# SciML/NeuralPDE.jl

Hardware: NVIDIA H100
Metric: collocation-points/sec (loss+grad) (higher is better)
Workload: dtype f32

## Files before the change

neuralpde.jl_b200/csrc/tc_kernel.cu:

```cuda
#include "tc_common.cuh"

namespace pinn {

using Fp = FpBlock<kTcW>;

struct CtaShared : CtaBase {
  int split, off_Q;
  uint8_t* stash;
  TcNetSmem nets[PINN_MAX_NETS];
};

struct LoopCtx {
  uint32_t fp;
  uint32_t bt;
  uint32_t tP;
  uint32_t tQ;
  float* gb;
  float* gw;
  uint32_t taddr;
  int act, split, p, lane, g0, g1, flag;
  __device__ __forceinline__ LoopCtx(uint32_t fp_, uint32_t bt_, uint32_t tP_, uint32_t tQ_, const Tid& t, int act_, int ng,
                                     int flag_, int split_ = 0, float* gb_ = nullptr, float* gw_ = nullptr)
      : fp(fp_), bt(bt_), tP(tP_), tQ(tQ_), gb(gb_), gw(gw_), taddr(t.lane_addr), act(act_), split(split_), p(t.p), lane(t.lane),
        g0(t.hh * (ng / kNH)), g1((t.hh + 1) * (ng / kNH)), flag(flag_) {}
};

template <int N1, int N2, bool PURE, int AK>
__device__ __forceinline__ void l0_fwd_loop(const LoopCtx lc, const PassInfo<N1, N2> pi, const float* xp, float* up) {
  constexpr int C = 1 + N1 + N2;
  float x[PINN_MAX_IN], u[C];
#pragma unroll
  for (int k = 0; k < PINN_MAX_IN; ++k) x[k] = xp[k];
#pragma unroll
  for (int c = 0; c < C; ++c) u[c] = up[c];
#pragma unroll 1
  for (int g = lc.g0; g < lc.g1; ++g) {
    float h[C][GW];
#pragma unroll
    for (int i = 0; i < GW; i += 2) {
      float za[C], zb2[C];
      first_layer_elem<kTcW>(lc.fp, pi, x, g * GW + i, za);
      first_layer_elem<kTcW>(lc.fp, pi, x, g * GW + i + 1, zb2);
      P2 zz[C], hv[C];
#pragma unroll
      for (int c = 0; c < C; ++c) zz[c] = mk2(za[c], zb2[c]);
      chain_fwd<N1, N2, PURE, AK, P2>(lc.act, pi.ch, zz, hv);
#pragma unroll
      for (int c = 0; c < C; ++c) { h[c][i] = hv[c].v.x; h[c][i + 1] = hv[c].v.y; }
      if (lc.flag) {
        const float w0 = lds_f32(lc.fp + (Fp::WL + g * GW + i) * 4), w1 = lds_f32(lc.fp + (Fp::WL + g * GW + i + 1) * 4);
#pragma unroll
        for (int c = 0; c < C; ++c) u[c] = fmaf(w1, hv[c].v.y, fmaf(w0, hv[c].v.x, u[c]));
      }
    }
#pragma unroll
    for (int c = 0; c < C; ++c) store_half(lc.tP + c * kTileBytes, lc.tQ + c * kTileBytes, lc.p, g * GW, h[c], lc.split != 0);
  }
#pragma unroll
  for (int c = 0; c < C; ++c) up[c] = u[c];
}

template <int C, int NK, bool SPLIT>
__device__ __forceinline__ void fwd_mma(float (&d)[C][16], uint32_t sP, uint32_t sQ, uint32_t whi, uint32_t wlo) {
  const int wg = threadIdx.x >> 7;
  const uint32_t aoff = (wg & 1) * 8192u, boff = (wg >> 1) * 32u * 128u;
  const uint64_t dwhi = tc::make_desc(whi + boff, 0, 1024), dwlo = tc::make_desc(wlo + boff, 0, 1024);
  tc::wgmma_fence();
#pragma unroll
  for (int c = 0; c < C; ++c) {
    const uint64_t dahi = tc::make_desc(sP + c * kTileBytes + aoff, 0, 1024);
    const uint64_t dalo = tc::make_desc(sQ + c * kTileBytes + aoff, 0, 1024);
#pragma unroll
    for (int pr = 0; pr < (SPLIT ? 3 : 1); ++pr) {
      const uint64_t a = (pr == 2) ? dalo : dahi, b = (pr == 1) ? dwlo : dwhi;
#pragma unroll
      for (int k = 0; k < NK; ++k)
        tc::wgmma_n32<0, 0>(d[c], a + 2 * k, b + 2 * k, (pr | k) ? 1u : 0u);
    }
  }
  tc::wgmma_commit();
  tc::wgmma_wait0();
}
template <int C>
__device__ __forceinline__ void fwd_mma_any(float (&d)[C][16], uint32_t sP, uint32_t sQ, uint32_t whi, uint32_t wlo, int nk,
                                            bool split) {
  switch (nk * 2 + (split ? 1 : 0)) {
    case 2: fwd_mma<C, 1, false>(d, sP, sQ, whi, wlo); break;
    case 3: fwd_mma<C, 1, true>(d, sP, sQ, whi, wlo); break;
    case 4: fwd_mma<C, 2, false>(d, sP, sQ, whi, wlo); break;
    case 5: fwd_mma<C, 2, true>(d, sP, sQ, whi, wlo); break;
    case 6: fwd_mma<C, 3, false>(d, sP, sQ, whi, wlo); break;
    case 7: fwd_mma<C, 3, true>(d, sP, sQ, whi, wlo); break;
    case 8: fwd_mma<C, 4, false>(d, sP, sQ, whi, wlo); break;
    default: fwd_mma<C, 4, true>(d, sP, sQ, whi, wlo); break;
  }
}

template <int N1, int N2, bool PURE, int AK, int C>
__device__ __forceinline__ void tl_fwd_frag(const float (&d)[C][16], const LoopCtx lc, const Chan<N1, N2> ch, float* scratch) {
  const int wg = threadIdx.x >> 7, w = (threadIdx.x >> 5) & 3;
  const int row0 = 64 * (wg & 1) + 16 * w + (lc.lane >> 2);
  const int col0 = 32 * (wg >> 1) + 2 * (lc.lane & 3);
  float u[2][C];
#pragma unroll
  for (int r = 0; r < 2; ++r)
#pragma unroll
    for (int c = 0; c < C; ++c) u[r][c] = 0.f;
#pragma unroll
  for (int i = 0; i < 16; i += 2) {
    const int rh = (i >> 1) & 1;
    const int row = row0 + 8 * rh, col = col0 + 8 * (i >> 2);
    P2 zz[C], hv[C];
    zz[0] = mk2(d[0][i] + lds_f32(lc.bt + col * 4), d[0][i + 1] + lds_f32(lc.bt + (col + 1) * 4));
#pragma unroll
    for (int c = 1; c < C; ++c) zz[c] = mk2(d[c][i], d[c][i + 1]);
    chain_fwd<N1, N2, PURE, AK, P2>(lc.act, ch, zz, hv);
    const uint32_t off = tc::swz_off(row, col);
#pragma unroll
    for (int c = 0; c < C; ++c) {
      const uint32_t hx = tc::pack_bf16(hv[c].v.x, hv[c].v.y);
      asm volatile("st.shared.b32 [%0], %1;" ::"r"(lc.tP + c * kTileBytes + off), "r"(hx) : "memory");
      if (lc.split)
        asm volatile("st.shared.b32 [%0], %1;" ::"r"(lc.tQ + c * kTileBytes + off), "r"(bf16x2_lo(hv[c].v.x, hv[c].v.y, hx))
                     : "memory");
    }
    if (lc.flag) {
      const float w0 = lds_f32(lc.fp + (Fp::WL + col) * 4), w1 = lds_f32(lc.fp + (Fp::WL + col + 1) * 4);
#pragma unroll
      for (int c = 0; c < C; ++c) u[rh][c] = fmaf(w1, hv[c].v.y, fmaf(w0, hv[c].v.x, u[rh][c]));
    }
  }
  if (lc.flag) {
#pragma unroll
    for (int r = 0; r < 2; ++r)
#pragma unroll
      for (int c = 0; c < C; ++c) {
        float s = u[r][c];
        s += __shfl_xor_sync(0xffffffffu, s, 1);
        s += __shfl_xor_sync(0xffffffffu, s, 2);
        if ((lc.lane & 3) == 0) atomicAdd(&scratch[c * kTcPts + row0 + 8 * r], s);
      }
  }
}

template <int C, int NKO>
__device__ __forceinline__ void dgrad_mma(float (&d)[C][16], uint32_t sP, uint32_t whi) {
  const uint32_t poff = (threadIdx.x >> 7) * 32u * 128u;
  const uint64_t dw = tc::make_desc(whi, 0, 1024);
  tc::wgmma_fence();
#pragma unroll
  for (int c = 0; c < C; ++c) {
    const uint64_t dz = tc::make_desc(sP + c * kTileBytes + poff, 0, 1024);
#pragma unroll
    for (int k = 0; k < NKO; ++k)
      tc::wgmma_n32<1, 0>(d[c], dw + 128 * k, dz + 2 * k, k ? 1u : 0u);
  }
  tc::wgmma_commit();
  tc::wgmma_wait0();
}
template <int C>
__device__ __forceinline__ void dgrad_mma_any(float (&d)[C][16], uint32_t sP, uint32_t whi, int nko) {
  switch (nko) {
    case 1: dgrad_mma<C, 1>(d, sP, whi); break;
    case 2: dgrad_mma<C, 2>(d, sP, whi); break;
    case 3: dgrad_mma<C, 3>(d, sP, whi); break;
    default: dgrad_mma<C, 4>(d, sP, whi); break;
  }
}
template <int C>
__device__ __forceinline__ void wgrad_mma(float (&dw)[32], float (&db)[8], uint32_t sP, uint32_t sQ, uint32_t s_ones) {
  const uint32_t poff = (threadIdx.x >> 7) * 32u * 128u;
  const uint64_t d1 = tc::make_desc(s_ones, 0, 0);
  tc::wgmma_fence();
#pragma unroll
  for (int c = 0; c < C; ++c) {
    const uint64_t dh = tc::make_desc(sQ + c * kTileBytes + poff, 0, 1024), dz = tc::make_desc(sP + c * kTileBytes + poff, 0, 1024);
#pragma unroll
    for (int k = 0; k < 2; ++k) tc::wgmma_n64<1, 1>(dw, dh + 128 * k, dz + 128 * k, (c | k) ? 1u : 0u);
  }
  const uint64_t dz0 = tc::make_desc(sP + poff, 0, 1024);
#pragma unroll
  for (int k = 0; k < 2; ++k) tc::wgmma_n16<1, 1>(db, dz0 + 128 * k, d1, k ? 1u : 0u);
  tc::wgmma_commit();
  tc::wgmma_wait0();
}

template <int NF>
__device__ __forceinline__ void frag_store_rows(float* base, int ld, const float (&d)[NF]) {
  const int w = (threadIdx.x >> 5) & 3, lane = threadIdx.x & 31;
  const bool odd = (lane & 1) != 0;
  float* row = base + (16 * w + (lane >> 2) + (odd ? 8 : 0)) * ld + 4 * ((lane >> 1) & 1);
#pragma unroll
  for (int j = 0; j < NF / 4; ++j) {
    const float r0 = __shfl_xor_sync(0xffffffffu, odd ? d[4 * j] : d[4 * j + 2], 1);
    const float r1 = __shfl_xor_sync(0xffffffffu, odd ? d[4 * j + 1] : d[4 * j + 3], 1);
    *reinterpret_cast<float4*>(row + 8 * j) =
        odd ? make_float4(r0, r1, d[4 * j + 2], d[4 * j + 3]) : make_float4(d[4 * j], d[4 * j + 1], r0, r1);
  }
}

template <int N1, int N2, bool PURE, int AK, int C>
__device__ __forceinline__ void tl_bwd_frag(const float (&d)[C][16], const LoopCtx lc, const Chan<N1, N2> ch, const float* ubs) {
  const int wg = threadIdx.x >> 7, w = (threadIdx.x >> 5) & 3;
  const int row0 = 64 * (wg & 1) + 16 * w + (lc.lane >> 2);
  const int col0 = 32 * (wg >> 1) + 2 * (lc.lane & 3);
  const float* hbar = tc::s_acc + TM_X * kAccRows;
#pragma unroll
  for (int i = 0; i < 16; i += 2) {
    const int row = row0 + 8 * ((i >> 1) & 1), col = col0 + 8 * (i >> 2);
    P2 zz[C], hv[C], zv[C];
    zz[0] = mk2(d[0][i] + lds_f32(lc.bt + col * 4), d[0][i + 1] + lds_f32(lc.bt + (col + 1) * 4));
#pragma unroll
    for (int c = 1; c < C; ++c) zz[c] = mk2(d[c][i], d[c][i + 1]);
    if (lc.flag) {
      const float w0 = lds_f32(lc.fp + (Fp::WL + col) * 4), w1 = lds_f32(lc.fp + (Fp::WL + col + 1) * 4);
#pragma unroll
      for (int c = 0; c < C; ++c) {
        const float u = ubs[c * kTcPts + row];
        hv[c] = mk2(w0 * u, w1 * u);
      }
    } else {
#pragma unroll
      for (int c = 0; c < C; ++c) hv[c] = mk2(hbar[(c * 64 + col) * kAccRows + row], hbar[(c * 64 + col + 1) * kAccRows + row]);
    }
    chain_bwd<N1, N2, PURE, AK, P2>(lc.act, ch, zz, hv, zv);
    const uint32_t off = tc::swz_off(row, col);
#pragma unroll
    for (int c = 0; c < C; ++c)
      asm volatile("st.shared.b32 [%0], %1;" ::"r"(lc.tP + c * kTileBytes + off), "r"(tc::pack_bf16(zv[c].v.x, zv[c].v.y))
                   : "memory");
  }
}

template <int N1, int N2, bool PURE, int AK>
__device__ __forceinline__ void l0_bwd_store_loop(const LoopCtx lc, const PassInfo<N1, N2> pi, const float* xp) {
  constexpr int C = 1 + N1 + N2;
  float x[PINN_MAX_IN];
#pragma unroll
  for (int k = 0; k < PINN_MAX_IN; ++k) x[k] = xp[k];
#pragma unroll 1
  for (int g = lc.g0; g < lc.g1; ++g) {
    float hb[C][GWB];
#pragma unroll
    for (int c = 0; c < C; ++c) acc_ldg(lc.taddr + TM_X + c * 64 + g * GWB, hb[c]);
#pragma unroll
    for (int i = 0; i < GWB; i += 2) {
      float za[C], zb2[C];
      first_layer_elem<kTcW>(lc.fp, pi, x, g * GWB + i, za);
      first_layer_elem<kTcW>(lc.fp, pi, x, g * GWB + i + 1, zb2);
      P2 zz[C], hv[C], zv[C];
#pragma unroll
      for (int c = 0; c < C; ++c) { zz[c] = mk2(za[c], zb2[c]); hv[c] = mk2(hb[c][i], hb[c][i + 1]); }
      chain_bwd<N1, N2, PURE, AK, P2>(lc.act, pi.ch, zz, hv, zv);
#pragma unroll
      for (int c = 0; c <= N1; ++c) { hb[c][i] = zv[c].v.x; hb[c][i + 1] = zv[c].v.y; }
    }
#pragma unroll
    for (int c = 0; c <= N1; ++c) store_half(lc.tP + c * kTileBytes, lc.tP, lc.p, g * GWB, hb[c], false);
  }
}

template <int N1, int N2, bool PURE, int AK>
__device__ __forceinline__ void l0_bwd_loop(const LoopCtx lc, const PassInfo<N1, N2> pi, const float* xp, const float* ubp) {
  constexpr int C = 1 + N1 + N2;
  float x[PINN_MAX_IN], ub[C];
#pragma unroll
  for (int k = 0; k < PINN_MAX_IN; ++k) x[k] = xp[k];
#pragma unroll
  for (int c = 0; c < C; ++c) ub[c] = ubp[c];
  const int re = reduceg_elem(lc.lane);
  const bool rlead = reduceg_lead(lc.lane);
  const int n1w = pi.n1w;
#pragma unroll 1
  for (int g = lc.g0; g < lc.g1; ++g) {
    float hb[C][GW];
    if (!lc.flag) {
#pragma unroll
      for (int c = 0; c < C; ++c) acc_ldg(lc.taddr + TM_X + c * 64 + g * GW, hb[c]);
    } else {
#pragma unroll
      for (int i = 0; i < GW; ++i) {
        const float wl = lds_f32(lc.fp + (Fp::WL + g * GW + i) * 4);
#pragma unroll
        for (int c = 0; c < C; ++c) hb[c][i] = wl * ub[c];
      }
    }
    float zv0[GW], zvd[N1 > 0 ? N1 : 1][GW];
#pragma unroll
    for (int i = 0; i < GW; ++i) {
      float zz[C], hv[C], zv[C];
      first_layer_elem<kTcW>(lc.fp, pi, x, g * GW + i, zz);
#pragma unroll
      for (int c = 0; c < C; ++c) hv[c] = hb[c][i];
      chain_bwd<N1, N2, PURE, AK, float>(lc.act, pi.ch, zz, hv, zv);
      zv0[i] = zv[0];
#pragma unroll
      for (int jd = 0; jd < N1; ++jd) zvd[jd][i] = zv[1 + jd];
    }
    const float bs = warp_reduceg(zv0, lc.lane);
    if (rlead) atomicAdd(lc.gb + g * GW + re, bs);
#pragma unroll
    for (int k = 0; k < PINN_MAX_IN; ++k) {
      if (k < pi.d_in) {
        float gk[GW];
#pragma unroll
        for (int i = 0; i < GW; ++i) {
          float gg = zv0[i] * x[k];
#pragma unroll
          for (int jd = 0; jd < N1; ++jd) gg += (pi.dir1[jd] == k) ? zvd[jd][i] : 0.f;
          gk[i] = gg;
        }
        const float gs = warp_reduceg(gk, lc.lane);
        if (rlead) atomicAdd(lc.gw + g * GW + re + (long long)n1w * k, gs);
      }
    }
  }
}

template <int N1, int N2, bool PURE, int AK>
__device__ __noinline__ uint32_t net_forward(CtaShared* cs, const DevProblem* Pp, const DevTerm* tmp, int slot,
                                             int want_grad, uint32_t phase) {
  extern __shared__ __align__(1024) uint8_t smem[];
  constexpr int C = 1 + N1 + N2;
  const DevTerm& tm = *tmp;
  const int net_id = tm.used_net[slot];
  const DevNet& net = Pp->nets[net_id];
  const DevChan& dc = tm.chan[slot];
  const TcNetSmem ns = cs->nets[net_id];
  const float* fp = reinterpret_cast<const float*>(smem + ns.fp);
  uint8_t* tP = smem + cs->off_P;
  uint8_t* tQ = smem + cs->off_Q;
  const Misc ms = misc_of(smem + cs->off_misc, cs->mx_dim, cs->mx_taps);
  const uint32_t accm = 0;
  const bool split = cs->split != 0;
  PassInfo<N1, N2> pi;
  load_pass<N1, N2>(pi, net, dc);
  const int TL = pi.TL;
  const Tid t = tid_of();
  const int tid = t.tid, p = t.p;
  float x[PINN_MAX_IN];
#pragma unroll
  for (int k = 0; k < PINN_MAX_IN; ++k) x[k] = (k < pi.d_in) ? ms.Xs[dc.rows[k] * kTcPts + p] : 0.f;
  uint8_t* stash_slot = cs->stash + (size_t)slot * cs->tl_max * kTcMaxC * kTileBytes;

  dbg_mark(cs, 10);
  float u[C];
#pragma unroll
  for (int c = 0; c < C; ++c) u[c] = 0.f;
  if (tid < C * kTcPts / 4) reinterpret_cast<float4*>(ms.scratch)[tid] = make_float4(0.f, 0.f, 0.f, 0.f);
  {
    const LoopCtx lc(tc::smem_u32(fp), tc::smem_u32(fp), tc::smem_u32(tP), tc::smem_u32(tQ), t, net.acts[0], pi.n1w / GW, TL == 0, split);
    l0_fwd_loop<N1, N2, PURE, AK>(lc, pi, x, u);
  }
  for (int l = 1; l <= TL; ++l) {
    const int n_in = net.dims[l], n_out = net.dims[l + 1];
    const int act = net.acts[l];
    tc::fence_async_smem();
    __syncthreads();
    dbg_mark(cs, 11);
    if (want_grad && tid == 0) {
      for (int c = 0; c < C; ++c)
        tc::bulk_store(stash_slot + (size_t)(l - 1) * kTcMaxC * kTileBytes + (size_t)c * kTileBytes, tP + c * kTileBytes, kTileBytes);
      tc::bulk_commit();
    }
    float d[C][16];
    {
      const uint32_t sP = tc::smem_u32(tP), sQ = tc::smem_u32(tQ);
      const uint32_t whi = tc::smem_u32(smem + ns.w_hi[l - 1]), wlo = tc::smem_u32(smem + ns.w_lo[l - 1]);
      const int nk = n_in / 16;
      fwd_mma_any<C>(d, sP, sQ, whi, wlo, nk, split);
    }
    dbg_mark(cs, 13);
    if (want_grad && tid == 0) tc::bulk_wait_read0();
    __syncthreads();
    dbg_mark(cs, 14);
    const LoopCtx lc(tc::smem_u32(fp), tc::smem_u32(fp) + (Fp::BT + (l - 1) * 64) * 4, tc::smem_u32(tP), tc::smem_u32(tQ), t, act, 0, l == TL, split);
    tl_fwd_frag<N1, N2, PURE, AK, C>(d, lc, pi.ch, ms.scratch);
  }
  finish_forward<C>(cs, tm, slot, ms, fp + Fp::BL, t, u);
  return phase;
}

template <int N1, int N2, bool PURE, int AK>
__device__ __noinline__ uint32_t net_backward(CtaShared* cs, const DevProblem* Pp, const DevTerm* tmp, int slot,
                                              uint32_t phase) {
  extern __shared__ __align__(1024) uint8_t smem[];
  constexpr int C = 1 + N1 + N2;
  const DevTerm& tm = *tmp;
  const int net_id = tm.used_net[slot];
  const DevNet& net = Pp->nets[net_id];
  const DevChan& dc = tm.chan[slot];
  const TcNetSmem ns = cs->nets[net_id];
  const float* fp = reinterpret_cast<const float*>(smem + ns.fp);
  uint8_t* tP = smem + cs->off_P;
  uint8_t* tQ = smem + cs->off_Q;
  const Misc ms = misc_of(smem + cs->off_misc, cs->mx_dim, cs->mx_taps);
  const uint32_t accm = 0;
  float* partial = cs->partial;
  PassInfo<N1, N2> pi;
  load_pass<N1, N2>(pi, net, dc);
  const int L = pi.L, TL = pi.TL;
  const Tid t = tid_of();
  const int tid = t.tid, p = t.p;
  uint32_t ld_phase = (phase >> 1) & 1u;
  float x[PINN_MAX_IN];
#pragma unroll
  for (int k = 0; k < PINN_MAX_IN; ++k) x[k] = (k < pi.d_in) ? ms.Xs[dc.rows[k] * kTcPts + p] : 0.f;
  uint8_t* stash_slot = cs->stash + (size_t)slot * cs->tl_max * kTcMaxC * kTileBytes;

  dbg_mark(cs, 20);
  float ub[C];
  gather_ubar<C>(tm, slot, ms, p, ub);
  if (t.hh == 0) {
#pragma unroll
    for (int c = 0; c < C; ++c) ms.scratch[c * kTcPts + p] = ub[c];
  }
  last_layer_grad<C>(t, ub, pi.nL, partial + net.w_off[L - 1], partial + net.b_off[L - 1], tc::smem_u32(tQ), tc::smem_u32(tP),
                     kTileBytes, 0u, accm + TM_Y, kTcW);

  const uint32_t sP = tc::smem_u32(tP), sQ = tc::smem_u32(tQ);
  const int wg = tid >> 7;
  float* hand = tc::s_acc + TM_X * kAccRows;
  float* wpart = reinterpret_cast<float*>(tP);
  float* bpart = ms.scratch;
  static_assert(4 * 64 <= kTcMaxC * kTcPts, "the bias partials fit ms.scratch");
  for (int l = TL; l >= 1; --l) {
    const int n_in = net.dims[l], n_out = net.dims[l + 1];
    const int act = net.acts[l];
    float* gb = partial + net.b_off[l];
    float* gw = partial + net.w_off[l];
    const float* bt = fp + Fp::BT + (l - 1) * 64;
    const uint32_t whi = tc::smem_u32(smem + ns.w_hi[l - 1]);
    dbg_mark(cs, 21);
    if (tid == 0 && l == TL) {
      const uint8_t* src = stash_slot + (size_t)(l - 1) * kTcMaxC * kTileBytes;
      tc::mbar_arrive_expect_tx(ms.bar_ld, C * kTileBytes);
      for (int c = 0; c < C; ++c) tc::bulk_load(tQ + c * kTileBytes, src + (size_t)c * kTileBytes, kTileBytes, ms.bar_ld);
    }
    wait_bar(ms.bar_ld, ld_phase);
    dbg_mark(cs, 22);
    {
      float d[C][16];
      fwd_mma_any<C>(d, sQ, sQ, whi, whi, n_in / 16, false);
      __syncthreads();
      dbg_mark(cs, 24);
      const LoopCtx lc(tc::smem_u32(fp), tc::smem_u32(bt), sP, sQ, t, act, 0, l == TL);
      tl_bwd_frag<N1, N2, PURE, AK, C>(d, lc, pi.ch, ms.scratch);
    }
    tc::fence_async_smem();
    __syncthreads();
    dbg_mark(cs, 26);
    {
      float d[C][16];
      dgrad_mma_any<C>(d, sP, whi, n_out / 16);
#pragma unroll
      for (int c = 0; c < C; ++c) frag_store_rows(hand + c * 64 * kAccRows + 32 * wg, kAccRows, d[c]);
    }
    dbg_mark(cs, 27);
    {
      float dw[32], db[8];
      wgrad_mma<C>(dw, db, sP, sQ, tc::smem_u32(smem + cs->off_ones));
      __syncthreads();
      if (tid == 0 && l > 1) {
        const uint8_t* src = stash_slot + (size_t)(l - 2) * kTcMaxC * kTileBytes;
        tc::mbar_arrive_expect_tx(ms.bar_ld, C * kTileBytes);
        for (int c = 0; c < C; ++c) tc::bulk_load(tQ + c * kTileBytes, src + (size_t)c * kTileBytes, kTileBytes, ms.bar_ld);
      }
      frag_store_rows(wpart + wg * 64 * 64, 64, dw);
      if ((t.lane & 3) == 0) {
        const int o = 16 * (t.warp & 3) + (t.lane >> 2);
        bpart[wg * 64 + o] = db[0];
        bpart[wg * 64 + o + 8] = db[2];
      }
    }
    __syncthreads();
    dbg_mark(cs, 28);
#pragma unroll 1
    for (int e = tid; e < 64 * 64; e += kTcThreads) {
      const int k = e >> 6, o = e & 63;
      if (k < n_in && o < n_out) atomicAdd(gw + o + (long long)n_out * k, ((wpart[e] + wpart[4096 + e]) + wpart[8192 + e]) + wpart[12288 + e]);
    }
    if (tid < n_out) atomicAdd(gb + tid, ((bpart[tid] + bpart[64 + tid]) + bpart[128 + tid]) + bpart[192 + tid]);
  }

  {
    __syncthreads();
    dbg_mark(cs, 29);
    const int act0 = net.acts[0];
    float* gb0 = partial + net.b_off[0];
    float* gw0 = partial + net.w_off[0];
    if (TL == 0) {
      const LoopCtx lc(tc::smem_u32(fp), tc::smem_u32(fp), sP, sQ, t, act0, pi.n1w / GW, 1, 0, gb0, gw0);
      l0_bwd_loop<N1, N2, PURE, AK>(lc, pi, x, ub);
    } else {
      coord_tiles<N1>(t, sQ, x, pi.dir1, N2 > 0);
      const LoopCtx lc(tc::smem_u32(fp), tc::smem_u32(fp), sP, sQ, t, act0, pi.n1w / GWB, 0);
      l0_bwd_store_loop<N1, N2, PURE, AK>(lc, pi, x);
      layer0_grad<N1>(t, sP, kTileBytes, 0u, sQ, N2 > 0, accm + TM_Y, kTcW, pi.n1w, pi.d_in, gw0, gb0);
    }
  }
  __syncthreads();
  dbg_mark(cs, 30);
  return (ld_phase << 1) | (phase & 1u);
}


__global__ void __launch_bounds__(kTcThreads, 1) tc_loss_grad_kernel(const __grid_constant__ TcArgs args) {
  extern __shared__ __align__(1024) uint8_t smem[];
  __shared__ CtaShared cs;
  const int tid = threadIdx.x;
  const DevProblem* Pp = args.prob;
  const DevProblem& P = *Pp;
  const Misc ms = misc_of(smem + args.off_misc, args.mx_dim, args.mx_taps);
  float* partial = args.partial + (long long)blockIdx.x * args.partial_stride;
  const bool want_grad = (args.mode == 0);
  const float* theta = args.theta;
  const DbgSpan span = dbg_span_begin(args.dbg);

  for (long long i = (long long)tid * 32; i < args.n_theta; i += (long long)kTcThreads * 32) tc::prefetch_l2(theta + i);
  {
    const char* nets0 = reinterpret_cast<const char*>(&Pp->nets[0]);
    const char* terms0 = reinterpret_cast<const char*>(&Pp->terms[0]);
    const int nb_nets = args.n_nets * (int)sizeof(DevNet), nb_terms = args.n_terms * (int)sizeof(DevTerm);
    if (tid == 0) tc::prefetch_l2(Pp);
    for (int o = tid * 128; o < nb_nets; o += kTcThreads * 128) tc::prefetch_l2(nets0 + o);
    for (int o = tid * 128; o < nb_terms; o += kTcThreads * 128) tc::prefetch_l2(terms0 + o);
    const int tile = args.tile_begin + (int)blockIdx.x;
    if (tile < args.tile_end && tid < 32) {
      int ti = 0;
      while (ti + 1 < args.n_terms && tile >= args.dyn[ti + 1].tile0) ++ti;
      const long long p0 = (long long)(tile - args.dyn[ti].tile0) * kTcPts;
      const long long row_bytes = 4ll * args.term_dim[ti];
      const long long off = p0 * row_bytes + (long long)tid * 128;
      if (off < args.dyn[ti].n * row_bytes) tc::prefetch_l2(reinterpret_cast<const char*>(args.dyn[ti].pts) + off);
    }
  }
  if (tid == 0) {
    tc::mbar_init(ms.bar_ld, 1);
    tc::fence_barrier_init();
    cs.split = args.split; cs.off_Q = args.off_Q;
    cs.stash = args.stash + (long long)blockIdx.x * args.stash_per_cta;
    for (int k = 0; k < PINN_MAX_NETS; ++k) cs.nets[k] = args.nets[k];
    cta_base_init(cs, args, partial);
  }
  if (tid == 0) tc::s_acc = args.acc + (size_t)blockIdx.x * kAccCols * kAccRows;
  cta_setup(args, ms, partial, P.n_theta, want_grad);
  for (int kn = 0; kn < P.n_nets; ++kn) {
    const DevNet& net = P.nets[kn];
    const TcNetSmem& ns = args.nets[kn];
    if (ns.fp < 0) continue;
    stage_fp_block<kTcW>(reinterpret_cast<float*>(smem + ns.fp), net, theta);
    const int L = net.n_layers;
    {
      constexpr int kItMax = kTcMaxTL * 512 / kTcThreads;
      const int n_items = (L - 2) * 512;
      float w[kItMax][8];
#pragma unroll
      for (int it = 0; it < kItMax; ++it) {
        const int i = tid + it * kTcThreads;
        if (i < n_items) {
          const int l = 1 + i / 512, r = i & 511;
          const int o = r & 63, kc = r >> 6;
          const int n_in = net.dims[l], n_out = net.dims[l + 1];
          const long long woff = net.w_off[l];
#pragma unroll
          for (int e = 0; e < 8; ++e) {
            const int k = kc * 8 + e;
            w[it][e] = (o < n_out && k < n_in) ? __ldg(&theta[woff + o + (long long)n_out * k]) : 0.f;
          }
        }
      }
#pragma unroll
      for (int it = 0; it < kItMax; ++it) {
        const int i = tid + it * kTcThreads;
        if (i < n_items) {
          const int l = 1 + i / 512, r = i & 511;
          const int o = r & 63, kc = r >> 6;
          uint8_t* thi = smem + ns.w_hi[l - 1];
          uint8_t* tlo = smem + ns.w_lo[l - 1];
          const float* v = w[it];
          uint32_t h[4];
#pragma unroll
          for (int e = 0; e < 4; ++e) h[e] = tc::pack_bf16(v[2 * e], v[2 * e + 1]);
          *reinterpret_cast<uint4*>(thi + tc::swz_chunk(o, kc)) = make_uint4(h[0], h[1], h[2], h[3]);
          if (args.split)
            *reinterpret_cast<uint4*>(tlo + tc::swz_chunk(o, kc)) = make_uint4(
                bf16x2_lo(v[0], v[1], h[0]), bf16x2_lo(v[2], v[3], h[1]), bf16x2_lo(v[4], v[5], h[2]), bf16x2_lo(v[6], v[7], h[3]));
        }
      }
    }
  }
  tc::fence_async_smem();
  __syncthreads();
  dbg_mark(&cs, 2);
  uint32_t phase = 0;

  for (int tile = args.tile_begin + blockIdx.x; tile < args.tile_end; tile += gridDim.x) {
    if (tid >= 128 && tid < 128 + (int)((sizeof(DevNet) * PINN_MAX_NETS + 127) / 128))
      tc::prefetch_l1(reinterpret_cast<const char*>(&P.nets[0]) + (tid - 128) * 128);
    uint32_t ldp = (phase >> 1) & 1u;
    const TileRef tr = stage_tile(args, P, ms, tile, ldp);
    phase = (phase & 1u) | (ldp << 1);
    const DevTerm* tmp = &P.terms[tr.ti];
    const DevTerm& tm = *tmp;
    const int n_used = tm.n_used;
    dbg_mark(&cs, 3);

    for (int slot = 0; slot < n_used; ++slot) {
      const int k1 = tm.chan[slot].n1, k2 = tm.chan[slot].n2, pu = tm.chan[slot].pure;
      const int ak = args.net_ak[tm.used_net[slot]];
      PINN_TC_DISPATCH(kTcMaxC, k1, k2, pu, ak, (phase = net_forward<A1, A2, PU, AK>(&cs, Pp, tmp, slot, want_grad ? 1 : 0, phase)));
    }

    dbg_mark(&cs, 4);
    residual_step(args, P, tm, ms, tr, smem + args.off_Q, (size_t)args.off_Q_bytes, partial, want_grad);

    dbg_mark(&cs, 5);
    if (want_grad) {
      if (tid == 0) tc::bulk_wait0();
      __syncthreads();
      dbg_mark(&cs, 6);
      for (int slot = n_used - 1; slot >= 0; --slot) {
        const int k1 = tm.chan[slot].n1, k2 = tm.chan[slot].n2, pu = tm.chan[slot].pure;
        const int ak = args.net_ak[tm.used_net[slot]];
        if (n_used > 1) {
          PINN_TC_DISPATCH(kTcMaxC, k1, k2, pu, ak, (phase = net_forward<A1, A2, PU, AK>(&cs, Pp, tmp, slot, 0, phase)));
        }
        PINN_TC_DISPATCH(kTcMaxC, k1, k2, pu, ak, (phase = net_backward<A1, A2, PU, AK>(&cs, Pp, tmp, slot, phase)));
      }
    }
  }

  __syncthreads();
  dbg_mark(&cs, 7);
  cta_finish(args, cs, span, ms, P, want_grad);
}

size_t tc_misc_bytes(int mx_dim, int mx_taps) {
  return (size_t)mx_dim * kTcPts * 4 + 2 * (size_t)mx_taps * kTcPts * 4 + (size_t)kTcMaxC * kTcPts * 4 + kTcPts * 4 +
         PINN_MAX_TERMS * 8 + 16 + 16;
}

cudaError_t tc_launch(const TcArgs& a, int grid, size_t smem, cudaStream_t st) {
  return launch_fused_kernel<tc_loss_grad_kernel>(a, grid, kTcThreads, smem, st);
}

}
```

Measured before the change: 93.04 million.

## Split hidden-layer backward into two 64-point halves reusing tile buffers

Restructures the hidden-layer backward pass to process the 128 collocation points in two halves. Each half recomputes its forward pre-activations with narrower n16 wgmma, writes the backward z into the second half of the Q tile, and keeps hbar in a swizzled smem layout inside the freed P tile. The weight-gradient partials now use plain (vectorised float4) read-modify-write into the per-CTA partial buffer instead of atomics, and the layer-0 path for TL==0 is hoisted. The intent is to cut shared-memory footprint and the number of bulk-load bytes per step and to remove atomic traffic, at the cost of twice as many layer iterations and barriers.

```diff
diff --git a/neuralpde.jl_b200/csrc/tc_kernel.cu b/neuralpde.jl_b200/csrc/tc_kernel.cu
--- a/neuralpde.jl_b200/csrc/tc_kernel.cu
+++ b/neuralpde.jl_b200/csrc/tc_kernel.cu
@@ -143,46 +143,94 @@
   }
 }
 
+constexpr uint32_t kHalfBytes = kTileBytes / 2;
+
+template <int C, int NK>
+__device__ __forceinline__ void rec_mma(float (&d)[C][8], uint32_t sQ, uint32_t whi) {
+  const uint64_t dw = tc::make_desc(whi + (threadIdx.x >> 7) * 16u * 128u, 0, 1024);
+  tc::wgmma_fence();
+#pragma unroll
+  for (int c = 0; c < C; ++c) {
+    const uint64_t da = tc::make_desc(sQ + c * kTileBytes, 0, 1024);
+#pragma unroll
+    for (int k = 0; k < NK; ++k) tc::wgmma_n16<0, 0>(d[c], da + 2 * k, dw + 2 * k, k ? 1u : 0u);
+  }
+  tc::wgmma_commit();
+  tc::wgmma_wait0();
+}
+template <int C>
+__device__ __forceinline__ void rec_mma_any(float (&d)[C][8], uint32_t sQ, uint32_t whi, int nk) {
+  switch (nk) {
+    case 1: rec_mma<C, 1>(d, sQ, whi); break;
+    case 2: rec_mma<C, 2>(d, sQ, whi); break;
+    case 3: rec_mma<C, 3>(d, sQ, whi); break;
+    default: rec_mma<C, 4>(d, sQ, whi); break;
+  }
+}
 template <int C, int NKO>
-__device__ __forceinline__ void dgrad_mma(float (&d)[C][16], uint32_t sP, uint32_t whi) {
-  const uint32_t poff = (threadIdx.x >> 7) * 32u * 128u;
+__device__ __forceinline__ void dgrad_mma(float (&d)[C][8], uint32_t sQ, uint32_t whi) {
+  const uint32_t poff = kHalfBytes + (threadIdx.x >> 7) * 16u * 128u;
   const uint64_t dw = tc::make_desc(whi, 0, 1024);
   tc::wgmma_fence();
 #pragma unroll
   for (int c = 0; c < C; ++c) {
-    const uint64_t dz = tc::make_desc(sP + c * kTileBytes + poff, 0, 1024);
+    const uint64_t dz = tc::make_desc(sQ + c * kTileBytes + poff, 0, 1024);
 #pragma unroll
     for (int k = 0; k < NKO; ++k)
-      tc::wgmma_n32<1, 0>(d[c], dw + 128 * k, dz + 2 * k, k ? 1u : 0u);
+      tc::wgmma_n16<1, 0>(d[c], dw + 128 * k, dz + 2 * k, k ? 1u : 0u);
   }
   tc::wgmma_commit();
   tc::wgmma_wait0();
 }
 template <int C>
-__device__ __forceinline__ void dgrad_mma_any(float (&d)[C][16], uint32_t sP, uint32_t whi, int nko) {
+__device__ __forceinline__ void dgrad_mma_any(float (&d)[C][8], uint32_t sQ, uint32_t whi, int nko) {
   switch (nko) {
-    case 1: dgrad_mma<C, 1>(d, sP, whi); break;
-    case 2: dgrad_mma<C, 2>(d, sP, whi); break;
-    case 3: dgrad_mma<C, 3>(d, sP, whi); break;
-    default: dgrad_mma<C, 4>(d, sP, whi); break;
+    case 1: dgrad_mma<C, 1>(d, sQ, whi); break;
+    case 2: dgrad_mma<C, 2>(d, sQ, whi); break;
+    case 3: dgrad_mma<C, 3>(d, sQ, whi); break;
+    default: dgrad_mma<C, 4>(d, sQ, whi); break;
   }
 }
 template <int C>
-__device__ __forceinline__ void wgrad_mma(float (&dw)[32], float (&db)[8], uint32_t sP, uint32_t sQ, uint32_t s_ones) {
-  const uint32_t poff = (threadIdx.x >> 7) * 32u * 128u;
+__device__ __forceinline__ void wgrad_mma(float (&dw)[32], float (&db)[8], uint32_t sQ, uint32_t s_ones) {
+  const uint32_t poff = (threadIdx.x >> 7) * 16u * 128u;
   const uint64_t d1 = tc::make_desc(s_ones, 0, 0);
   tc::wgmma_fence();
 #pragma unroll
   for (int c = 0; c < C; ++c) {
-    const uint64_t dh = tc::make_desc(sQ + c * kTileBytes + poff, 0, 1024), dz = tc::make_desc(sP + c * kTileBytes + poff, 0, 1024);
-#pragma unroll
-    for (int k = 0; k < 2; ++k) tc::wgmma_n64<1, 1>(dw, dh + 128 * k, dz + 128 * k, (c | k) ? 1u : 0u);
-  }
-  const uint64_t dz0 = tc::make_desc(sP + poff, 0, 1024);
-#pragma unroll
-  for (int k = 0; k < 2; ++k) tc::wgmma_n16<1, 1>(db, dz0 + 128 * k, d1, k ? 1u : 0u);
+    const uint64_t dh = tc::make_desc(sQ + c * kTileBytes + poff, 0, 1024);
+    const uint64_t dz = tc::make_desc(sQ + c * kTileBytes + kHalfBytes + poff, 0, 1024);
+    tc::wgmma_n64<1, 1>(dw, dh, dz, c ? 1u : 0u);
+  }
+  tc::wgmma_n16<1, 1>(db, tc::make_desc(sQ + kHalfBytes + poff, 0, 1024), d1, 0u);
   tc::wgmma_commit();
   tc::wgmma_wait0();
+}
+
+__device__ __forceinline__ int hb_idx(int c, int k, int p) { return (c * 64 + k) * 64 + (p ^ ((((k >> 1) ^ k) & 3) << 3)); }
+
+template <int C>
+__device__ __forceinline__ void hbar_store(float* hbar, const float (&d)[C][8]) {
+  const int wg = threadIdx.x >> 7, w = (threadIdx.x >> 5) & 3, lane = threadIdx.x & 31;
+#pragma unroll
+  for (int c = 0; c < C; ++c)
+#pragma unroll
+    for (int i = 0; i < 8; i += 2) {
+      const int k = 16 * w + (lane >> 2) + 8 * ((i >> 1) & 1), p = 16 * wg + 8 * (i >> 2) + 2 * (lane & 3);
+      *reinterpret_cast<float2*>(hbar + hb_idx(c, k, p)) = make_float2(d[c][i], d[c][i + 1]);
+    }
+}
+
+template <int C>
+__device__ __forceinline__ void hbar0_store(float* hand, const float (&d)[C][8], int h) {
+  const int wg = threadIdx.x >> 7, w = (threadIdx.x >> 5) & 3, lane = threadIdx.x & 31;
+#pragma unroll
+  for (int c = 0; c < C; ++c)
+#pragma unroll
+    for (int i = 0; i < 8; i += 2) {
+      const int k = 16 * w + (lane >> 2) + 8 * ((i >> 1) & 1), p = 64 * h + 16 * wg + 8 * (i >> 2) + 2 * (lane & 3);
+      *reinterpret_cast<float2*>(hand + (c * 64 + k) * kAccRows + p) = make_float2(d[c][i], d[c][i + 1]);
+    }
 }
 
 template <int NF>
@@ -200,13 +248,13 @@
 }
 
 template <int N1, int N2, bool PURE, int AK, int C>
-__device__ __forceinline__ void tl_bwd_frag(const float (&d)[C][16], const LoopCtx lc, const Chan<N1, N2> ch, const float* ubs) {
+__device__ __forceinline__ void tl_bwd_frag(const float (&d)[C][8], const LoopCtx lc, const Chan<N1, N2> ch, const float* ubs,
+                                            const float* hbar, int h) {
   const int wg = threadIdx.x >> 7, w = (threadIdx.x >> 5) & 3;
-  const int row0 = 64 * (wg & 1) + 16 * w + (lc.lane >> 2);
-  const int col0 = 32 * (wg >> 1) + 2 * (lc.lane & 3);
-  const float* hbar = tc::s_acc + TM_X * kAccRows;
-#pragma unroll
-  for (int i = 0; i < 16; i += 2) {
+  const int row0 = 16 * w + (lc.lane >> 2);
+  const int col0 = 16 * wg + 2 * (lc.lane & 3);
+#pragma unroll
+  for (int i = 0; i < 8; i += 2) {
     const int row = row0 + 8 * ((i >> 1) & 1), col = col0 + 8 * (i >> 2);
     P2 zz[C], hv[C], zv[C];
     zz[0] = mk2(d[0][i] + lds_f32(lc.bt + col * 4), d[0][i + 1] + lds_f32(lc.bt + (col + 1) * 4));
@@ -216,18 +264,18 @@
       const float w0 = lds_f32(lc.fp + (Fp::WL + col) * 4), w1 = lds_f32(lc.fp + (Fp::WL + col + 1) * 4);
 #pragma unroll
       for (int c = 0; c < C; ++c) {
-        const float u = ubs[c * kTcPts + row];
+        const float u = ubs[c * kTcPts + 64 * h + row];
         hv[c] = mk2(w0 * u, w1 * u);
       }
     } else {
 #pragma unroll
-      for (int c = 0; c < C; ++c) hv[c] = mk2(hbar[(c * 64 + col) * kAccRows + row], hbar[(c * 64 + col + 1) * kAccRows + row]);
+      for (int c = 0; c < C; ++c) hv[c] = mk2(hbar[hb_idx(c, col, row)], hbar[hb_idx(c, col + 1, row)]);
     }
     chain_bwd<N1, N2, PURE, AK, P2>(lc.act, ch, zz, hv, zv);
-    const uint32_t off = tc::swz_off(row, col);
+    const uint32_t off = kHalfBytes + tc::swz_off(row, col);
 #pragma unroll
     for (int c = 0; c < C; ++c)
-      asm volatile("st.shared.b32 [%0], %1;" ::"r"(lc.tP + c * kTileBytes + off), "r"(tc::pack_bf16(zv[c].v.x, zv[c].v.y))
+      asm volatile("st.shared.b32 [%0], %1;" ::"r"(lc.tQ + c * kTileBytes + off), "r"(tc::pack_bf16(zv[c].v.x, zv[c].v.y))
                    : "memory");
   }
 }
@@ -274,16 +322,11 @@
 #pragma unroll 1
   for (int g = lc.g0; g < lc.g1; ++g) {
     float hb[C][GW];
-    if (!lc.flag) {
-#pragma unroll
-      for (int c = 0; c < C; ++c) acc_ldg(lc.taddr + TM_X + c * 64 + g * GW, hb[c]);
-    } else {
-#pragma unroll
-      for (int i = 0; i < GW; ++i) {
-        const float wl = lds_f32(lc.fp + (Fp::WL + g * GW + i) * 4);
-#pragma unroll
-        for (int c = 0; c < C; ++c) hb[c][i] = wl * ub[c];
-      }
+#pragma unroll
+    for (int i = 0; i < GW; ++i) {
+      const float wl = lds_f32(lc.fp + (Fp::WL + g * GW + i) * 4);
+#pragma unroll
+      for (int c = 0; c < C; ++c) hb[c][i] = wl * ub[c];
     }
     float zv0[GW], zvd[N1 > 0 ? N1 : 1][GW];
 #pragma unroll
@@ -419,86 +462,110 @@
                      kTileBytes, 0u, accm + TM_Y, kTcW);
 
   const uint32_t sP = tc::smem_u32(tP), sQ = tc::smem_u32(tQ);
+  const int act0 = net.acts[0];
+  float* gb0 = partial + net.b_off[0];
+  float* gw0 = partial + net.w_off[0];
+  if (TL == 0) {
+    __syncthreads();
+    dbg_mark(cs, 29);
+    const LoopCtx lc(tc::smem_u32(fp), tc::smem_u32(fp), sP, sQ, t, act0, pi.n1w / GW, 1, 0, gb0, gw0);
+    l0_bwd_loop<N1, N2, PURE, AK>(lc, pi, x, ub);
+  }
+
   const int wg = tid >> 7;
+  float* hbar = reinterpret_cast<float*>(tP);
+  float* wpart = reinterpret_cast<float*>(tP);
+  float* bpart = reinterpret_cast<float*>(tQ + kHalfBytes);
   float* hand = tc::s_acc + TM_X * kAccRows;
-  float* wpart = reinterpret_cast<float*>(tP);
-  float* bpart = ms.scratch;
-  static_assert(4 * 64 <= kTcMaxC * kTcPts, "the bias partials fit ms.scratch");
-  for (int l = TL; l >= 1; --l) {
-    const int n_in = net.dims[l], n_out = net.dims[l + 1];
-    const int act = net.acts[l];
-    float* gb = partial + net.b_off[l];
-    float* gw = partial + net.w_off[l];
-    const float* bt = fp + Fp::BT + (l - 1) * 64;
-    const uint32_t whi = tc::smem_u32(smem + ns.w_hi[l - 1]);
-    dbg_mark(cs, 21);
-    if (tid == 0 && l == TL) {
-      const uint8_t* src = stash_slot + (size_t)(l - 1) * kTcMaxC * kTileBytes;
-      tc::mbar_arrive_expect_tx(ms.bar_ld, C * kTileBytes);
-      for (int c = 0; c < C; ++c) tc::bulk_load(tQ + c * kTileBytes, src + (size_t)c * kTileBytes, kTileBytes, ms.bar_ld);
-    }
-    wait_bar(ms.bar_ld, ld_phase);
-    dbg_mark(cs, 22);
-    {
-      float d[C][16];
-      fwd_mma_any<C>(d, sQ, sQ, whi, whi, n_in / 16, false);
+#pragma unroll 1
+  for (int h = 0; h < (TL > 0 ? 2 : 0); ++h) {
+    for (int l = TL; l >= 1; --l) {
+      const int n_in = net.dims[l], n_out = net.dims[l + 1];
+      const int act = net.acts[l];
+      float* gb = partial + net.b_off[l];
+      float* gw = partial + net.w_off[l];
+      const float* bt = fp + Fp::BT + (l - 1) * 64;
+      const uint32_t whi = tc::smem_u32(smem + ns.w_hi[l - 1]);
+      dbg_mark(cs, 21);
+      if (tid == 0 && l == TL) {
+        const uint8_t* src = stash_slot + (size_t)(l - 1) * kTcMaxC * kTileBytes + h * kHalfBytes;
+        tc::mbar_arrive_expect_tx(ms.bar_ld, C * kHalfBytes);
+        for (int c = 0; c < C; ++c) tc::bulk_load(tQ + c * kTileBytes, src + (size_t)c * kTileBytes, kHalfBytes, ms.bar_ld);
+      }
+      wait_bar(ms.bar_ld, ld_phase);
+      dbg_mark(cs, 22);
+      {
+        float d[C][8];
+        rec_mma_any<C>(d, sQ, whi, n_in / 16);
+        __syncthreads();
+        dbg_mark(cs, 24);
+        const LoopCtx lc(tc::smem_u32(fp), tc::smem_u32(bt), sP, sQ, t, act, 0, l == TL);
+        tl_bwd_frag<N1, N2, PURE, AK, C>(d, lc, pi.ch, ms.scratch, hbar, h);
+      }
+      tc::fence_async_smem();
       __syncthreads();
-      dbg_mark(cs, 24);
-      const LoopCtx lc(tc::smem_u32(fp), tc::smem_u32(bt), sP, sQ, t, act, 0, l == TL);
-      tl_bwd_frag<N1, N2, PURE, AK, C>(d, lc, pi.ch, ms.scratch);
-    }
-    tc::fence_async_smem();
-    __syncthreads();
-    dbg_mark(cs, 26);
-    {
-      float d[C][16];
-      dgrad_mma_any<C>(d, sP, whi, n_out / 16);
-#pragma unroll
-      for (int c = 0; c < C; ++c) frag_store_rows(hand + c * 64 * kAccRows + 32 * wg, kAccRows, d[c]);
-    }
-    dbg_mark(cs, 27);
-    {
-      float dw[32], db[8];
-      wgrad_mma<C>(dw, db, sP, sQ, tc::smem_u32(smem + cs->off_ones));
+      dbg_mark(cs, 26);
+      float db0, db2;
+      {
+        float dw[32], db[8];
+        wgrad_mma<C>(dw, db, sQ, tc::smem_u32(smem + cs->off_ones));
+        frag_store_rows(wpart + wg * 64 * 64, 64, dw);
+        db0 = db[0]; db2 = db[2];
+      }
+      float d[C][8];
+      dgrad_mma_any<C>(d, sQ, whi, n_out / 16);
       __syncthreads();
+      dbg_mark(cs, 27);
       if (tid == 0 && l > 1) {
-        const uint8_t* src = stash_slot + (size_t)(l - 2) * kTcMaxC * kTileBytes;
-        tc::mbar_arrive_expect_tx(ms.bar_ld, C * kTileBytes);
-        for (int c = 0; c < C; ++c) tc::bulk_load(tQ + c * kTileBytes, src + (size_t)c * kTileBytes, kTileBytes, ms.bar_ld);
-      }
-      frag_store_rows(wpart + wg * 64 * 64, 64, dw);
+        const uint8_t* src = stash_slot + (size_t)(l - 2) * kTcMaxC * kTileBytes + h * kHalfBytes;
+        tc::mbar_arrive_expect_tx(ms.bar_ld, C * kHalfBytes);
+        for (int c = 0; c < C; ++c) tc::bulk_load(tQ + c * kTileBytes, src + (size_t)c * kTileBytes, kHalfBytes, ms.bar_ld);
+      }
       if ((t.lane & 3) == 0) {
         const int o = 16 * (t.warp & 3) + (t.lane >> 2);
-        bpart[wg * 64 + o] = db[0];
-        bpart[wg * 64 + o + 8] = db[2];
-      }
-    }
-    __syncthreads();
-    dbg_mark(cs, 28);
+        bpart[wg * 64 + o] = db0;
+        bpart[wg * 64 + o + 8] = db2;
+      }
+      __syncthreads();
+      dbg_mark(cs, 28);
+      if ((reinterpret_cast<uintptr_t>(gw) & 15) == 0) {
+        const float4* wp4 = reinterpret_cast<const float4*>(wpart);
 #pragma unroll 1
-    for (int e = tid; e < 64 * 64; e += kTcThreads) {
-      const int k = e >> 6, o = e & 63;
-      if (k < n_in && o < n_out) atomicAdd(gw + o + (long long)n_out * k, ((wpart[e] + wpart[4096 + e]) + wpart[8192 + e]) + wpart[12288 + e]);
-    }
-    if (tid < n_out) atomicAdd(gb + tid, ((bpart[tid] + bpart[64 + tid]) + bpart[128 + tid]) + bpart[192 + tid]);
-  }
-
-  {
+        for (int e = tid; e < 64 * 16; e += kTcThreads) {
+          const int k = e >> 4, o = (e & 15) * 4;
+          if (k < n_in && o < n_out) {
+            const float4 a = wp4[e], b = wp4[1024 + e], c = wp4[2048 + e], q = wp4[3072 + e];
+            float4* g = reinterpret_cast<float4*>(gw + o + (long long)n_out * k);
+            float4 v = *g;
+            v.x += ((a.x + b.x) + c.x) + q.x;
+            v.y += ((a.y + b.y) + c.y) + q.y;
+            v.z += ((a.z + b.z) + c.z) + q.z;
+            v.w += ((a.w + b.w) + c.w) + q.w;
+            *g = v;
+          }
+        }
+      } else {
+#pragma unroll 1
+        for (int e = tid; e < 64 * 64; e += kTcThreads) {
+          const int k = e >> 6, o = e & 63;
+          if (k < n_in && o < n_out) gw[o + (long long)n_out * k] += ((wpart[e] + wpart[4096 + e]) + wpart[8192 + e]) + wpart[12288 + e];
+        }
+      }
+      if (tid < n_out) gb[tid] += ((bpart[tid] + bpart[64 + tid]) + bpart[128 + tid]) + bpart[192 + tid];
+      __syncthreads();
+      if (l > 1) hbar_store<C>(hbar, d);
+      else hbar0_store<C>(hand, d, h);
+    }
+  }
+  if (TL > 0) {
     __syncthreads();
     dbg_mark(cs, 29);
-    const int act0 = net.acts[0];
-    float* gb0 = partial + net.b_off[0];
-    float* gw0 = partial + net.w_off[0];
-    if (TL == 0) {
-      const LoopCtx lc(tc::smem_u32(fp), tc::smem_u32(fp), sP, sQ, t, act0, pi.n1w / GW, 1, 0, gb0, gw0);
-      l0_bwd_loop<N1, N2, PURE, AK>(lc, pi, x, ub);
-    } else {
-      coord_tiles<N1>(t, sQ, x, pi.dir1, N2 > 0);
-      const LoopCtx lc(tc::smem_u32(fp), tc::smem_u32(fp), sP, sQ, t, act0, pi.n1w / GWB, 0);
-      l0_bwd_store_loop<N1, N2, PURE, AK>(lc, pi, x);
-      layer0_grad<N1>(t, sP, kTileBytes, 0u, sQ, N2 > 0, accm + TM_Y, kTcW, pi.n1w, pi.d_in, gw0, gb0);
-    }
-  }
+    coord_tiles<N1>(t, sQ, x, pi.dir1, N2 > 0);
+    const LoopCtx lc(tc::smem_u32(fp), tc::smem_u32(fp), sP, sQ, t, act0, pi.n1w / GWB, 0);
+    l0_bwd_store_loop<N1, N2, PURE, AK>(lc, pi, x);
+    layer0_grad<N1>(t, sP, kTileBytes, 0u, sQ, N2 > 0, accm + TM_Y, kTcW, pi.n1w, pi.d_in, gw0, gb0);
+  }
+
   __syncthreads();
   dbg_mark(cs, 30);
   return (ld_phase << 1) | (phase & 1u);
```

Result: faster. 98.06 million, median of 6 (+5.4%).
